# Tomsk-Smart-Tech/video-stream-segmenetation

Measured on AMD Instinct MI355X. Metric: frames/sec (640×480, batch=8) at 1/2/4/8 MI355X + mask max-abs-err vs ref, higher is better.
Workload: dtype bf16; 1 GPU; 8 synthetic 640x480 RGB u8 frames per GPU per step (resident in HBM) -> 256x144 f32 masks, 4 steps in flight (one handle, 4 slots, 4 streams); global_batch=8, frame=640x480x3, model_res=256x144, pw_gemm=v_mfma_f32_16x16x32_bf16, f32 activations split hi+lo, graph=True, inflight=4, parallelism=dp1

## Files before the change

### video-stream-segmenetation_amd/csrc/vss_kernels.h

```cpp
#pragma once
#include <cstddef>
#include <cstdint>

#include <hip/hip_runtime.h>

namespace vss {

enum Prec : int { PREC_F32 = 0, PREC_BF16X2 = 1, PREC_BF16 = 2 };

enum BlockMode : int { MODE_IR_EXPAND = 0, MODE_IR_DIRECT = 1, MODE_DEC = 2 };

__host__ __device__ constexpr int block_flags(int norm_in, int residual, int xp, int sp, int ks, int stem_in = 0) {
  return (norm_in ? 1 : 0) | (residual ? 2 : 0) | ((xp - 1) << 2) | ((sp - 1) << 4) | ((ks - 1) << 6) |
         (stem_in ? 256 : 0);
}
__host__ __device__ constexpr bool flags_stem_in(int f) { return (f & 256) != 0; }
__host__ __device__ constexpr int flags_xp(int f) { return ((f >> 2) & 3) + 1; }
__host__ __device__ constexpr int flags_sp(int f) { return ((f >> 4) & 3) + 1; }
__host__ __device__ constexpr int flags_ks(int f) { return ((f >> 6) & 3) + 1; }

constexpr int kThreads = 256;
constexpr int kLdsGranule = 2048, kLdsGranulesPerCu = 80;
__host__ __device__ constexpr int lds_wg_per_cu(int bytes) {
  return kLdsGranulesPerCu / ((bytes + kLdsGranule - 1) / kLdsGranule);
}
constexpr int kMaxAcc = 16;
#ifndef VSS_PERM
#define VSS_PERM 0
#endif
#ifndef VSS_XS_PAD
#define VSS_XS_PAD 4
#endif
#ifndef VSS_HS1
#define VSS_HS1 20
#endif
#ifndef VSS_QUADS
#define VSS_QUADS 1
#endif
__host__ __device__ constexpr int block_pix(int r) { return VSS_PERM ? (r < 4 ? r : (r < 12 ? r + 4 : r - 8)) : r; }
__host__ __device__ constexpr int hid_stride(int stride) { return stride == 2 ? 20 : VSS_HS1; }

#ifndef VSS_SWZ
#define VSS_SWZ 1
#endif
__host__ __device__ constexpr int pow2div16(int q) {
  return q % 16 == 0 ? 16 : (q % 8 == 0 ? 8 : (q % 4 == 0 ? 4 : (q % 2 == 0 ? 2 : 1)));
}
__host__ __device__ constexpr int gray_swz(int pix, int m) { return (pix ^ (pix >> 1)) & (m - 1); }
constexpr int kAccSlots = 4;

__host__ __device__ constexpr int r4(int v) { return (v + 3) & ~3; }
__host__ __device__ constexpr int cmax(int a, int b) { return a > b ? a : b; }

__host__ __device__ constexpr int dw_run(int TW, int NPB, int PW) {
  return (TW % 4 == 0 && 16 % (TW / 4) == 0 && NPB % 4 == 0 && (NPB / 4) % PW == 0)   ? 4
         : (TW % 2 == 0 && 16 % (TW / 2) == 0 && NPB % 2 == 0 && (NPB / 2) % PW == 0) ? 2
                                                                                      : 1;
}

struct BlockLds {
  int IH, IW, P_in, P_in_pad, P_out, CX, XS, LD2, SR, SC;
  bool XQM;
  int XPL, XSW, HPL, RS, RSW, XRW;
  int NCB, NPB, NCHUNK, PW, CS, NPBW, NACC;
  int xt, xr, w1, w2, wdw, bdw, b2, wimg_end, lr, nrm, uc, work, stt, total;
  int slab_stride;
  int slab;
};

__host__ __device__ constexpr int stem_xwp(int IW) {
  if (!VSS_SWZ) return 2 * IW + 2;
  const int xw = 2 * IW + 1, hw2 = IW + 1;
  int x = xw;
  while ((x - hw2) % 32 != 0) ++x;
  return x;
}
__host__ __device__ constexpr int stem_in_lds(int IH, int IW) {
  return r4(3 * (2 * IH + 1) * stem_xwp(IW)) + 27 * 16 + 16;
}

__host__ __device__ constexpr BlockLds block_lds(int mode, int stride, int TH, int TW, int cin, int cskip, int chid,
                                                 int cout, int stem_in = 0) {
  BlockLds L{};
  L.IH = stride == 2 ? 2 * TH + 1 : TH + 2;
  L.IW = stride == 2 ? 2 * TW + 1 : TW + 2;
  L.P_in = L.IH * L.IW;
  L.P_in_pad = (L.P_in + 15) & ~15;
  L.P_out = TH * TW;
  L.CX = mode == 2  ? cin + cskip : cin;
  L.XQM = VSS_SWZ && mode == 1;
  L.XS = !VSS_SWZ ? L.CX + VSS_XS_PAD : (L.XQM ? 4 : (mode == 2 ? L.CX + (TW == 16 ? 8 : VSS_XS_PAD) : L.CX));
  L.XPL = L.XQM ? 4 * L.P_in_pad : 0;
  L.XSW = VSS_SWZ && mode == 0 ? pow2div16(L.CX / 4) : 1;

  L.RS = VSS_SWZ ? cout : cout + 4;
  L.RSW = VSS_SWZ ? pow2div16(cout / 4) : 1;
  L.XRW = VSS_SWZ ? pow2div16(cin / 4) : 1;
  L.LD2 = chid + 8;
  L.SR = (TH + 1) / 2 + 3;
  L.SC = (TW + 1) / 2 + 3;
  L.NCB = cout / 16;
  L.NPB = L.P_out / 16;
  L.NCHUNK = chid / 16;
  L.CS = L.NCHUNK >= 4 ? 4 : (L.NCHUNK >= 2 ? 2 : 1);
  L.PW = 4 / L.CS;
  L.NPBW = L.NPB / L.PW;
  L.NACC = L.NPBW * L.NCB;
  L.HPL = VSS_SWZ && mode == 0 && dw_run(TW, L.NPB, 1) == 1 ? 4 * (L.P_in_pad + (stride == 2 ? 1 : 0)) : 0;
  L.slab_stride = L.P_out * L.RS;
  const int xt_floats = L.XQM ? L.P_in_pad * L.CX : r4(L.P_in_pad * L.XS);
  int o = 0;
  L.xt = o;  o += xt_floats;
  L.xr = o;  o += (mode == 0 && stride == 1 && cin == cout) ? r4(L.P_out * cin) : 0;
  L.w1 = o;
  L.w2 = o;  o += mode == 0 ? 0 : r4(cout * L.LD2 / 2);
  L.wdw = o; o += mode == 0 ? 0 : r4(9 * chid);
  L.bdw = o; o += mode == 0 ? 0 : r4(chid);
  L.b2 = o;  o += r4(cout);
  L.wimg_end = o;
  const bool slab_in_xt = mode == 2 && L.CS * L.slab_stride <= xt_floats;
  const bool dec_quads = mode == 2 && VSS_QUADS && TH % 2 == 0 && TW % 2 == 0;
  L.work = o;
  L.lr = o;
  const int hid_floats = L.HPL ? 4 * 4 * L.HPL : 4 * L.P_in_pad * hid_stride(stride);
  o += cmax(cmax(cmax(mode == 0 ? hid_floats : 1024, slab_in_xt ? 0 : L.CS * L.slab_stride),
                 mode == 2 && !dec_quads ? r4(L.SR * L.SC * cin) : 0),
            stem_in ? stem_in_lds(L.IH, L.IW) : 0);
  L.nrm = o; o += mode == 2 ? r4(2 * cin) : 0;
  L.uc = o;  o += (mode == 2 && !dec_quads) ? 4 * L.P_in_pad : 0;
  L.slab = slab_in_xt ? L.xt : L.work;
  L.stt = slab_in_xt ? L.work : L.xt;
  L.total = o;
  return L;
}

struct ExpandFrag {
  int NK, NCB, aw, f4s, a2, bytes;
};
constexpr int kFragF4 = 11;
__host__ __device__ constexpr ExpandFrag expand_frag(int cin, int cout) {
  ExpandFrag F{};
  F.NK = cin / 16;
  F.NCB = cout / 16;
  F.aw = 0;
  F.f4s = F.aw + 512 * F.NK;
  F.a2 = F.f4s + kFragF4 * 64;
  F.bytes = F.a2 + 512 * F.NCB;
  return F;
}
__host__ __device__ constexpr int frag_off(int n, int i, int l) {
  return (n % 2 == 1 && i == n - 1) ? (n / 2) * 1024 + l * 8 : (i / 2) * 1024 + l * 16 + (i % 2) * 8;
}

#ifdef VSS_TRACE
#define VSS_TRACE_FIELD unsigned long long* trace;
#define VSS_STAMP(k)                                                                                  \
  do {                                                                                                \
    if constexpr (!COH) {                                                                             \
      if (threadIdx.x == 0 && p.trace) {                                                              \
        unsigned long long* t_ = p.trace + (((long)blockIdx.z * gridDim.y + blockIdx.y) * gridDim.x + blockIdx.x) * 16; \
        t_[(k)] = __builtin_amdgcn_s_memrealtime();                                                   \
        t_[8 + (k)] = __builtin_amdgcn_s_memtime();                                                   \
        if ((k) == 0) {                                                                               \
                                    \
          t_[7] = __builtin_amdgcn_s_getreg((31 << 11) | 4);                                          \
          t_[15] = __builtin_amdgcn_s_getreg((15 << 11) | 20);                                        \
        }                                                                                             \
      }                                                                                               \
    }                                                                                                 \
  } while (0)
#else
#define VSS_TRACE_FIELD
#define VSS_STAMP(k) \
  do {               \
  } while (0)
#endif

struct StemParams {
  const uint8_t* frames;
  long row_stride, frame_stride;
  int fh, fw, fc;
  int Hm, Wm;
  float ry, rx;
  const float* w;
  const float* b;
  float* y;
  int Ho, Wo, cout;
  unsigned long long* acc_zero;
  int acc_stride;
  VSS_TRACE_FIELD
};

struct BlockParams {
  const float* wimg;
  long wimg_stride;
  const char* wfrag;
// ... 440 lines not shown
```

### video-stream-segmenetation_amd/csrc/vss_kernels.hip

```cpp
#include <hip/hip_runtime.h>

#include <vector>

#include "vss_kernels.h"

namespace vss {

typedef float f4 __attribute__((ext_vector_type(4)));
typedef unsigned u4 __attribute__((ext_vector_type(4)));
typedef __bf16 bf4 __attribute__((ext_vector_type(4)));
typedef __bf16 bf8 __attribute__((ext_vector_type(8)));

__device__ __forceinline__ const void* uniform_ptr(const void* p) {
  const unsigned long long v = reinterpret_cast<unsigned long long>(p);
  const unsigned lo = __builtin_amdgcn_readfirstlane((unsigned)v);
  const unsigned hi = __builtin_amdgcn_readfirstlane((unsigned)(v >> 32));
  return reinterpret_cast<const void*>(((unsigned long long)hi << 32) | lo);
}

template <bool COH>
struct Gm {
  const float* b;
  __amdgpu_buffer_rsrc_t r;
  __device__ __forceinline__ explicit Gm(const float* base) : b(base) {
// ... 433 lines not shown
    }
  }
};

#ifndef VSS_WDMA
#define VSS_WDMA 1
#endif
#ifndef VSS_WDMA_ALL
#define VSS_WDMA_ALL 0
#endif
#ifndef VSS_WDMA_FIRST
#define VSS_WDMA_FIRST 0
#endif
constexpr bool block_wdma(int mode, int wimg_f4) {
  return VSS_WDMA && (VSS_WDMA_ALL || mode == 2 || wimg_f4 >= 2560);
}
template <int N>
__device__ __forceinline__ void dma_f4(const f4* src, f4* dst) {
  const int lane = (int)threadIdx.x & 63;
  const int wb = __builtin_amdgcn_readfirstlane(((int)threadIdx.x >> 6) * 64);
  for (int o = wb; o < N; o += 256)
    if (N % 64 == 0 || o + lane < N)
      __builtin_amdgcn_global_load_lds((__attribute__((address_space(1))) void*)(src + o + lane),
                                       (__attribute__((address_space(3))) void*)(dst + o), 16, 0, 0);
}
struct NoStaged {
  template <class Load>
  __device__ __forceinline__ void issue(Load) {}
  template <class Store>
  __device__ __forceinline__ void commit(Store) const {}
};
template <bool ON>
__device__ __forceinline__ void dma_wait() {
  if constexpr (ON) asm volatile("s_waitcnt vmcnt(0)" ::: "memory");
}

template <bool B>
struct ChunkTag {
  static constexpr bool value = B;
};

template <int MODE, int STRIDE, int TH, int TW, int CIN, int CSKIP, int CH, int COUT, int FLAGS, int PREC, bool COH>
__device__ __forceinline__ void block_body(const BlockParams& p, int bx, int by, int bz, float* smem) {
  constexpr bool STEM_IN = flags_stem_in(FLAGS);
  constexpr BlockLds L = block_lds(MODE, STRIDE, TH, TW, CIN, CSKIP, CH, COUT, STEM_IN);
  constexpr bool NORM_IN = (FLAGS & 1) != 0, RES = (FLAGS & 2) != 0;
  constexpr int XP = flags_xp(FLAGS), SP = flags_sp(FLAGS), KS = flags_ks(FLAGS);
  static_assert(KS == 1 || MODE == MODE_IR_EXPAND, "only expand layers split their hidden channels");
  static_assert(SP == 1 || MODE == MODE_DEC, "skip parts: decoder only");
  constexpr int IW = L.IW, P_IN = L.P_in, P_IN_PAD = L.P_in_pad, P_OUT = L.P_out, XS = L.XS;
  constexpr int NCB = L.NCB, NPB = L.NPB, NCHUNK = L.NCHUNK, PW = L.PW, CS = L.CS, NPBW = L.NPBW;
  constexpr int RS = L.RS, SS = L.slab_stride;
  static_assert(L.NACC <= kMaxAcc, "too many accumulators per wave");
  static_assert(CIN % 16 == 0 && CH % 16 == 0 && COUT % 16 == 0 && P_OUT % 16 == 0, "shape");
  static_assert(MODE != MODE_IR_EXPAND || CIN <= 64, "expand cin <= 64");
  static_assert(!RES || (STRIDE == 1 && CIN == COUT && MODE != MODE_DEC), "residual shape");
  static_assert(MODE != MODE_IR_EXPAND || CS == 4, "expand deals its chunks to the 4 waves");
  static_assert(NPB % PW == 0, "pixel blocks must split evenly over the wave groups");
  constexpr int XT_FLOATS = L.XQM ? P_IN_PAD * L.CX : r4(P_IN_PAD * XS);
  static_assert(MODE != MODE_DEC || (XT_FLOATS >= (NORM_IN ? kAccSlots * 2 * CIN * 2 : 0) &&
                                     (L.slab == L.xt ? L.stt == L.work : (L.stt == L.xt && XT_FLOATS >= 1024))),
                "decoder: xt holds the src's norm slots (prologue); the stats scratch (epilogue) sits in the "
                "work region when the slabs take xt, else in xt");
  const int tid = threadIdx.x, lane = tid & 63, wave = tid >> 6;
  const int r = lane & 15, g = lane >> 4;
  const int n = KS == 1 ? bz : bz / KS;
  const int ks = KS == 1 ? 0 : bz % KS;
  const int oy0 = by * TH, ox0 = bx * TW;
  const int iy0 = STRIDE * oy0 - 1, ix0 = STRIDE * ox0 - 1;
  const int Ho = p.Ho, Wo = p.Wo;
  float* xt = smem + L.xt;
  const uint16_t* w2s = reinterpret_cast<const uint16_t*>(smem + L.w2);
  const float* wdws = smem + L.wdw;
  const float* bdws = smem + L.bdw;
  const float* b2s = smem + L.b2;
  float* work = smem + L.work;
  float* slabs = smem + L.slab;
  float* stt = smem + L.stt;
  auto xq = [&](int pix, int q) {
    if constexpr (L.XQM) return q * L.XPL + 4 * pix;
    else return pix * XS + 4 * (q ^ gray_swz(pix, L.XSW));
  };
  auto sq = [&](int sl, int pix, int q) { return sl * SS + pix * RS + 4 * (q ^ gray_swz(pix, L.RSW)); };
  auto rq = [&](int pix, int q) { return pix * CIN + 4 * (q ^ (pix & (L.XRW - 1))); };
  constexpr bool EXPAND = MODE == MODE_IR_EXPAND;
  constexpr ExpandFrag F = expand_frag(CIN, COUT);
  const char* frag = EXPAND ? p.wfrag + ks * p.wfrag_stride : nullptr;
  const int wave_u = __builtin_amdgcn_readfirstlane(wave);
  FragRegs<EXPAND ? F.NK : 1> w1f;
  f4 b1f;
  auto load_w1 = [&](int ck) {
    const char* rec = frag + ck * F.bytes;
    w1f.load(rec + F.aw, lane);
    b1f = *reinterpret_cast<const f4*>(rec + F.f4s + g * 16);
  };
  VSS_STAMP(0);

  constexpr int WIMG_F4 = (L.wimg_end - L.w1) / 4;
  constexpr bool WDMA = block_wdma(MODE, WIMG_F4);
  const f4* wsrc = reinterpret_cast<const f4*>(p.wimg + ks * p.wimg_stride);
  f4* wdst = reinterpret_cast<f4*>(smem + L.w1);
  if constexpr (MODE == MODE_DEC) {
    constexpr int CL = CIN, C4L = CL / 4, SR = L.SR, SC = L.SC;
    const int h = p.H, w = p.W;
    float* lr = smem + L.lr;
    float* nrm = smem + L.nrm;
    const int sy0 = max(0, (oy0 - 1) / 2 - 1), sx0 = max(0, (ox0 - 1) / 2 - 1);
    const float* xn = p.x + (long)n * h * w * CL;
    const float* sn = p.skip + (long)n * Ho * Wo * CSKIP;
    constexpr int NSLOT16 = NORM_IN ? kAccSlots * 2 * CL / 2 : 0;
    Staged<NSLOT16> st_slots;
    const Gm<COH> g_slots(reinterpret_cast<const float*>(p.in_acc + (long)n * p.acc_stride));
    if constexpr (NORM_IN) st_slots.issue([&](int i) { return g_slots.ld(4L * i); });
    static_assert(CL % 16 == 0 && CSKIP % 16 == 0, "16-channel staging items");
    constexpr int GL = CL / 16, GS = CSKIP / 16;
    constexpr bool QUADS = VSS_QUADS && TH % 2 == 0 && TW % 2 == 0;
    constexpr int QH = L.IH / 2, QW = IW / 2, NQI = QH * QW * C4L, NQ = QUADS ? (NQI + 255) / 256 : 0;
    Staged16<QUADS ? 0 : SR * SC * GL, XP, VSS_STAGE16_DEC> st_lr;
    f4 tap[XP][NQ > 0 ? NQ : 1][4];
    Staged16<P_IN_PAD * GS, SP, VSS_STAGE16_DEC> st_sk;
    constexpr bool SKP = VSS_SWZ && GS == 1 && !L.XQM && VSS_STAGE16_DEC == 0 && (XS / 4) % 4 == 2;
    auto skip_pix = [&](int it) { return SKP ? (it & ~3) | ((it & 1) << 1) | ((it >> 1) & 1) : it; };
    std::conditional_t<WDMA, NoStaged, Staged<WIMG_F4>> st_w;
    {
      const float* xb[XP];
#pragma unroll
      for (int q = 0; q < XP; ++q) xb[q] = xn + q * p.x_part_stride;
      if constexpr (QUADS) {
        const int j0 = (iy0 - 1) / 2, i0 = (ix0 - 1) / 2;
#pragma unroll
        for (int k = 0; k < NQ; ++k) {
          const int it = min(tid + 256 * k, NQI - 1);
          const int c4 = it % C4L, qq = it / C4L, qx = qq % QW, qy = qq / QW;
          const int ya = min(max(j0 + qy, 0), h - 1), yb = min(max(j0 + qy + 1, 0), h - 1);
          const int ca = min(max(i0 + qx, 0), w - 1), cb = min(max(i0 + qx + 1, 0), w - 1);
          const unsigned o[4] = {(unsigned)((ya * w + ca) * CL + 4 * c4), (unsigned)((ya * w + cb) * CL + 4 * c4),
                                 (unsigned)((yb * w + ca) * CL + 4 * c4), (unsigned)((yb * w + cb) * CL + 4 * c4)};
#pragma unroll
          for (int q = 0; q < XP; ++q)
#pragma unroll
            for (int t = 0; t < 4; ++t)
              tap[q][k][t] = *reinterpret_cast<const f4*>(reinterpret_cast<const char*>(xb[q]) + (o[t] << 2));
        }
      } else {
        st_lr.issue(xb, [&](int i) {
          const int pr = i / GL, gq = i - pr * GL;
          const int yy = min(h - 1, sy0 + pr / SC), xx = min(w - 1, sx0 + pr % SC);
          return (unsigned)((yy * w + xx) * CL + 16 * gq);
        });
      }
      const float* sb[SP];
#pragma unroll
      for (int q = 0; q < SP; ++q) sb[q] = sn + q * p.skip_part_stride;
      st_sk.issue(sb, [&](int i) {
        const int pix = skip_pix(i / GS), gq = i - (i / GS) * GS, py = pix / IW;
        const int yy = min(max(iy0 + py, 0), Ho - 1), xx = min(max(ix0 + pix - py * IW, 0), Wo - 1);
        return (unsigned)((yy * Wo + xx) * CSKIP + 16 * gq);
      });
    }
    if constexpr (WDMA) dma_f4<WIMG_F4>(wsrc, reinterpret_cast<f4*>(smem + L.w1));
    st_w.issue([&](int i) { return wsrc[i]; });
    VSS_STAMP(6);
    static_assert(SR * SC * CL < 65536, "tap offsets are u16");
    unsigned* uc = reinterpret_cast<unsigned*>(smem + L.uc);
    if constexpr (!QUADS)
    for (int pix = tid; pix < P_IN_PAD; pix += 256) {
      const int yy = iy0 + pix / IW, xx = ix0 + pix % IW;
// ... 176 lines not shown
        const unsigned x1 = (unsigned)min(sp.fw - 1, (int)ceilf(fx));
        dxs[u][e] = fx - x0f;
        const unsigned o0 = (unsigned)x0f * (unsigned)sp.fc, o1 = x1 * (unsigned)sp.fc;
#pragma unroll
        for (int c = 0; c < 3; ++c) {
          raw[u][e][c] = __builtin_amdgcn_raw_buffer_load_b8(frsrc, (int)(t0 + o0) + c, 0, 0);
          raw[u][e][3 + c] = __builtin_amdgcn_raw_buffer_load_b8(frsrc, (int)(t0 + o1) + c, 0, 0);
          raw[u][e][6 + c] = __builtin_amdgcn_raw_buffer_load_b8(frsrc, (int)(t1 + o0) + c, 0, 0);
          raw[u][e][9 + c] = __builtin_amdgcn_raw_buffer_load_b8(frsrc, (int)(t1 + o1) + c, 0, 0);
        }
      }
    }
    VSS_STAMP(6);
#pragma unroll
    for (int u = 0; u < NR; ++u) {
      float o[2][3];
      prep_finish2(raw[u][0], raw[u][1], dys[u], dxs[u][0], dys[u], dxs[u][1], o[0], o[1]);
      const int ly = lys[u], yy = r0 + ly;
#pragma unroll
      for (int e = 0; e < 2; ++e) {
        const int lx = lxs[u] + e * HW2, xx = c0 + lx;
        const bool in = tid + 256 * u < NPAIR && lx < XW;
        const bool valid = ((unsigned)yy < (unsigned)sp.Hm) & ((unsigned)xx < (unsigned)sp.Wm);
        if (in) {
#pragma unroll
          for (int c = 0; c < 3; ++c) x0s[(c * XH + ly) * XWP + lx] = valid ? o[e][c] : 0.f;
        }
      }
    }
#pragma unroll
    for (int u = 0; u < 2; ++u) {
      const int i = tid + 256 * u;
      if (i < 27 * 16) sws[i] = wr[u];
    }
    if (tid < 16) sbs[tid] = sb;
    if (bx == 0 && by == 0)
      for (int i = tid; i < sp.acc_stride; i += 256) {
        if constexpr (COH)
          __hip_atomic_store(sp.acc_zero + (long)n * sp.acc_stride + i, 0ull, __ATOMIC_RELAXED, __HIP_MEMORY_SCOPE_AGENT);
        else
          sp.acc_zero[(long)n * sp.acc_stride + i] = 0ull;
      }
    st_w.commit([&](int i, f4 v) { wdst[i] = v; });
    VSS_STAMP(4);
    dma_wait<WDMA>();
    __syncthreads();
    VSS_STAMP(5);
    {
      const StemTaps taps = stem_taps<XH * XWP, XWP>(sws, r, g);
      if constexpr (VSS_SWZ) {
        const f4 bias4 = *reinterpret_cast<const f4*>(sbs + 4 * g);
        for (int blk = wave; blk < P_IN_PAD / 16; blk += 4) {
          const int pa = min(blk * 16 + r, P_IN - 1), py = pa / IW, px = pa - py * IW;
          const f4 acc = stem_mfma_t(taps, x0s + 2 * py * XWP + 2 * px, bias4);
          *reinterpret_cast<f4*>(xt + xq(blk * 16 + r, g)) = relu6v(acc);
        }
      } else {
        const float bias = sbs[r];
        for (int blk = wave; blk < P_IN_PAD / 16; blk += 4) {
          const int pa = min(blk * 16 + r, P_IN - 1), py = pa / IW, px = pa - py * IW;
          const f4 acc = stem_mfma(taps, x0s + 2 * py * XWP + 2 * px, bias);
          const int p0 = blk * 16 + 4 * g;
#pragma unroll
          for (int i = 0; i < 4; ++i) xt[xq(p0 + i, r >> 2) + (r & 3)] = relu6f(acc[i]);
        }
      }
      const bool interior = iy0 >= 0 && iy0 + L.IH <= H && ix0 >= 0 && ix0 + IW <= W;
      if (!interior) {
        __syncthreads();
        for (int i = tid; i < P_IN * 4; i += 256) {
          const int q = L.XQM ? i / P_IN : i & 3, e = L.XQM ? i - q * P_IN : i >> 2, qy = e / IW, qx = e - qy * IW;
          const int yy = iy0 + qy, xx = ix0 + qx;
          if (yy < 0 || yy >= H || xx < 0 || xx >= W)
            *reinterpret_cast<f4*>(xt + xq(qy * IW + qx, q)) = f4{0.f, 0.f, 0.f, 0.f};
        }
      }
    }

  } else {
    const int H = p.H, W = p.W;
    const float* xn = p.x + (long)n * H * W * CIN;
    static_assert(CIN % 16 == 0, "16-channel staging items");
    constexpr int GI = CIN / 16;
    Staged16<P_IN_PAD * GI, XP, VSS_STAGE16> st_x;
    std::conditional_t<WDMA, NoStaged, Staged<WIMG_F4>> st_w;
    if constexpr (WDMA && VSS_WDMA_FIRST) dma_f4<WIMG_F4>(wsrc, reinterpret_cast<f4*>(smem + L.w1));
    {
      const float* xb[XP];
#pragma unroll
      for (int q = 0; q < XP; ++q) xb[q] = xn + q * p.x_part_stride;
      st_x.issue(xb, [&](int i) {
        const int pix = i / GI, gq = i - pix * GI, py = pix / IW;
        const int yy = min(max(iy0 + py, 0), H - 1), xx = min(max(ix0 + pix - py * IW, 0), W - 1);
        return (unsigned)((yy * W + xx) * CIN + 16 * gq);
      });
    }
    if constexpr (WDMA && !VSS_WDMA_FIRST) dma_f4<WIMG_F4>(wsrc, reinterpret_cast<f4*>(smem + L.w1));
    st_w.issue([&](int i) { return wsrc[i]; });
    if constexpr (EXPAND) load_w1(wave_u);
    VSS_STAMP(6);
    st_x.commit_sum([&](int i, int k, f4 v) {
      const int pix = i / GI, c4 = (i - pix * GI) * 4 + k;
      if constexpr (MODE == MODE_IR_EXPAND) {
        *reinterpret_cast<f4*>(xt + xq(pix, c4)) = to_operand<PREC>(v);
        if constexpr (RES) {
          const int py = pix / IW, px = pix - py * IW;
          if (py >= 1 && py <= TH && px >= 1 && px <= TW)
            *reinterpret_cast<f4*>(smem + L.xr + rq((py - 1) * TW + px - 1, c4)) = v;
        }
      } else {
        const int py = pix / IW, px = pix % IW;
        const int yy = iy0 + py, xx = ix0 + px;
        const bool valid = pix < P_IN && yy >= 0 && yy < H && xx >= 0 && xx < W;
        *reinterpret_cast<f4*>(xt + xq(pix, c4)) = valid ? v : f4{0.f, 0.f, 0.f, 0.f};
      }
    });
    st_w.commit([&](int i, f4 v) { wdst[i] = v; });
    VSS_STAMP(4);
  }
  dma_wait<WDMA>();
  __syncthreads();
  VSS_STAMP(1);

  f4 acc[L.NACC];
  const int pw = wave % PW, cw = wave / PW;
  constexpr int XR = dw_run(TW, NPB, MODE == MODE_IR_EXPAND ? 1 : PW);
  static_assert(NPB % XR == 0 && NPBW % XR == 0, "dw runs");
  auto run_pix = [&](int sb, int j) {
    if constexpr (XR == 1) return sb * 16 + block_pix(r);
    else return (sb * (16 * XR / TW) + r / (TW / XR)) * TW + (r % (TW / XR)) * XR + j;
  };

  if constexpr (MODE == MODE_IR_EXPAND) {
    constexpr int HSD = hid_stride(STRIDE);
    float* hid = work + wave * (L.HPL ? 4 * L.HPL : P_IN_PAD * HSD);
    auto hq = [&](int pix, int q) {
      if constexpr (L.HPL != 0) return q * L.HPL + 4 * pix;
      else return pix * HSD + 4 * q;
    };
    constexpr int NK = CIN / 16;
    constexpr int NCBI = P_IN_PAD / 16;
    static_assert(NCBI <= 32, "one validity bit per input pixel block");
    unsigned vmask = ~0u;
    if (!(iy0 >= 0 && iy0 + L.IH <= p.H && ix0 >= 0 && ix0 + IW <= p.W)) {
      vmask = 0u;
#pragma unroll
      for (int cb = 0; cb < NCBI; ++cb) {
        const int pix = cb * 16 + r, py = pix / IW, yy = iy0 + py, xx = ix0 + pix - py * IW;
        vmask |= (yy >= 0 && yy < p.H && xx >= 0 && xx < p.W) ? 1u << cb : 0u;
      }
    }
    auto expand_chunk = [&](int ck, auto first) {
      constexpr bool FIRST = decltype(first)::value;
      const char* rec = frag + ck * F.bytes;
      f4 wk[9];
#pragma unroll
      for (int t = 0; t < 9; ++t) wk[t] = *reinterpret_cast<const f4*>(rec + F.f4s + (4 * (1 + t) + g) * 16);
      const f4 bb = *reinterpret_cast<const f4*>(rec + F.f4s + (4 * 10 + g) * 16);
      FragRegs<NCB> w2f;
      w2f.load(rec + F.a2, lane);
      typename AFrag<PREC>::T aw[NK];
#pragma unroll
      for (int s = 0; s < NK; ++s) aw[s] = frag_a<PREC>(w1f.v[s]);
      const f4 bias = b1f;
      constexpr int UNRL = block_lds(MODE, STRIDE, TH, TW, CIN, CSKIP, CH, COUT, STEM_IN).P_in_pad / 16 <= 6
                               ? block_lds(MODE, STRIDE, TH, TW, CIN, CSKIP, CH, COUT, STEM_IN).P_in_pad / 16
                               : 2;
#pragma unroll UNRL
      for (int cb = 0; cb < NCBI; ++cb) {
        const int pix = cb * 16 + r;
        f4 d = bias;
#pragma unroll
        for (int s = 0; s < NK; ++s) d = mma16_op<PREC>(d, aw[s], *reinterpret_cast<const f4*>(xt + xq(pix, 4 * s + g)));
        *reinterpret_cast<f4*>(hid + hq(pix, g)) = clampv(d, (vmask >> cb) & 1u ? 6.f : 0.f);
      }
      wave_sync();
      {
        if constexpr (NCHUNK > 4) load_w1(min(ck + 4, NCHUNK - 1));
        typename AFrag<PREC>::T a2[NCB];
#pragma unroll
        for (int cb = 0; cb < NCB; ++cb) a2[cb] = frag_a<PREC>(w2f.v[cb]);
#pragma unroll
        for (int q = 0; q < NPB / XR; ++q) {
          const int pix0 = run_pix(q, 0), ly = pix0 / TW, lx0 = pix0 % TW;
          f4 a[XR];
#pragma unroll
          for (int j = 0; j < XR; ++j) a[j] = bb;
#pragma unroll
          for (int ky = 0; ky < 3; ++ky) {
            constexpr int NT = STRIDE * (XR - 1) + 3;
            f4 t[NT];
#pragma unroll
            for (int u = 0; u < NT; ++u)
              t[u] = *reinterpret_cast<const f4*>(hid + hq((STRIDE * ly + ky) * IW + STRIDE * lx0 + u, g));
#pragma unroll
            for (int j = 0; j < XR; ++j)
#pragma unroll
              for (int kx = 0; kx < 3; ++kx) a[j] = __builtin_elementwise_fma(wk[ky * 3 + kx], t[STRIDE * j + kx], a[j]);
          }
#pragma unroll
          for (int j = 0; j < XR; ++j) {
            const f4 b = to_operand<PREC>(relu6v(a[j]));
#pragma unroll
            for (int cb = 0; cb < NCB; ++cb) {
              f4& ac = acc[(q * XR + j) * NCB + cb];
              if constexpr (FIRST)
                ac = mma16_op<PREC>(f4{0.f, 0.f, 0.f, 0.f}, a2[cb], b);
              else
                ac = mma16_op<PREC>(ac, a2[cb], b);
            }
          }
        }
      }
      wave_sync();
    };
    static_assert(NCHUNK >= 4, "every wave has a first chunk");
    expand_chunk(wave_u, ChunkTag<true>{});
    for (int ck = wave_u + 4; ck < NCHUNK; ck += 4) expand_chunk(ck, ChunkTag<false>{});
  } else {
    auto dw_chunk = [&](int ck, auto first) {
      constexpr bool FIRST = decltype(first)::value;
      const int c0 = ck << 4;
      f4 wk[9];
#pragma unroll
      for (int t = 0; t < 9; ++t) wk[t] = *reinterpret_cast<const f4*>(wdws + t * CH + c0 + 4 * g);
      const f4 bb = *reinterpret_cast<const f4*>(bdws + c0 + 4 * g);
      typename AFrag<PREC>::T a2[NCB];
#pragma unroll
      for (int cb = 0; cb < NCB; ++cb) a2[cb] = lds_a<PREC>(w2s, L.LD2, cb * 16 + r, c0 + 4 * g);
#pragma unroll
      for (int q = 0; q < NPBW / XR; ++q) {
        const int pix0 = run_pix(pw + q * PW, 0), ly = pix0 / TW, lx0 = pix0 % TW;
        f4 a[XR];
#pragma unroll
        for (int j = 0; j < XR; ++j) a[j] = bb;
#pragma unroll
        for (int ky = 0; ky < 3; ++ky) {
          f4 t[XR + 2];
#pragma unroll
          for (int u = 0; u < XR + 2; ++u)
            t[u] = *reinterpret_cast<const f4*>(xt + xq((ly + ky) * IW + lx0 + u, (c0 >> 2) + g));
#pragma unroll
          for (int j = 0; j < XR; ++j)
#pragma unroll
            for (int kx = 0; kx < 3; ++kx) a[j] = __builtin_elementwise_fma(wk[ky * 3 + kx], t[j + kx], a[j]);
        }
#pragma unroll
        for (int j = 0; j < XR; ++j) {
          if constexpr (MODE == MODE_IR_DIRECT) a[j] = relu6v(a[j]);
          const f4 b = to_operand<PREC>(a[j]);
#pragma unroll
          for (int cb = 0; cb < NCB; ++cb) {
            f4& ac = acc[(q * XR + j) * NCB + cb];
            if constexpr (FIRST)
              ac = mma16_op<PREC>(f4{0.f, 0.f, 0.f, 0.f}, a2[cb], b);
            else
              ac = mma16_op<PREC>(ac, a2[cb], b);
          }
        }
      }
    };
    static_assert(CS <= NCHUNK, "every wave has a first chunk");
    dw_chunk(cw, ChunkTag<true>{});
    for (int ck = cw + CS; ck < NCHUNK; ck += CS) dw_chunk(ck, ChunkTag<false>{});
  }

  if constexpr (MODE == MODE_IR_DIRECT && CS == 1) {
    VSS_STAMP(2);
    const Gm<COH> gy(p.y + (long)n * Ho * Wo * COUT);
#pragma unroll
    for (int q = 0; q < NPBW / XR; ++q)
#pragma unroll
      for (int j = 0; j < XR; ++j) {
        const int pix = run_pix(pw + q * PW, j), ly = pix / TW, lx = pix % TW;
        const int oy = oy0 + ly, ox = ox0 + lx;
#pragma unroll
        for (int cb = 0; cb < NCB; ++cb) {
          f4 v = acc[(q * XR + j) * NCB + cb] + *reinterpret_cast<const f4*>(b2s + cb * 16 + 4 * g);
          if constexpr (RES) v = v + *reinterpret_cast<const f4*>(xt + xq((ly + 1) * IW + lx + 1, cb * 4 + g));
          if (oy < Ho && ox < Wo) gy.st(((long)oy * Wo + ox) * COUT + cb * 16 + 4 * g, v);
        }
      }
  } else {
  __syncthreads();
  VSS_STAMP(2);
  {
#pragma unroll
    for (int q = 0; q < NPBW / XR; ++q)
#pragma unroll
      for (int j = 0; j < XR; ++j)
#pragma unroll
        for (int cb = 0; cb < NCB; ++cb)
          *reinterpret_cast<f4*>(slabs + sq(cw, run_pix(pw + q * PW, j), cb * 4 + g)) = acc[(q * XR + j) * NCB + cb];
  }
  __syncthreads();
  constexpr int C4O = COUT / 4, NOUT = (P_OUT * C4O + 255) / 256;
  const Gm<COH> gy(p.y + ks * p.y_part_stride + (long)n * Ho * Wo * COUT);
  f4 outv[MODE == MODE_DEC ? NOUT : 1];
#pragma unroll
  for (int k = 0; k < NOUT; ++k) {
    const int i = tid + 256 * k;
    if (i < P_OUT * C4O) {
      const int pix = i / C4O, c4 = i % C4O;
      const int ly = pix / TW, lx = pix % TW;
      const int oy = oy0 + ly, ox = ox0 + lx;
      const bool valid = oy < Ho && ox < Wo;
      f4 v = *reinterpret_cast<const f4*>(slabs + sq(0, pix, c4));
#pragma unroll
      for (int s = 1; s < CS; ++s) v = v + *reinterpret_cast<const f4*>(slabs + sq(s, pix, c4));
      if (KS == 1 || ks == 0) {
        v = v + *reinterpret_cast<const f4*>(b2s + 4 * c4);
        if constexpr (RES) {
          if constexpr (MODE == MODE_IR_EXPAND)
            v = v + *reinterpret_cast<const f4*>(smem + L.xr + rq(pix, c4));
          else
            v = v + *reinterpret_cast<const f4*>(xt + xq((ly + 1) * IW + lx + 1, c4));
        }
      }
      if constexpr (MODE == MODE_DEC) {
        outv[k] = v;
        *reinterpret_cast<f4*>(slabs + sq(0, pix, c4)) = valid ? v : f4{0.f, 0.f, 0.f, 0.f};
      } else if (valid) {
        gy.st(((long)oy * Wo + ox) * COUT + 4 * c4, v);
      }
    }
  }
  if constexpr (MODE == MODE_DEC) {
    __syncthreads();
    constexpr int G = 256 / COUT;
    static_assert((P_OUT + G - 1) / G <= 16, "f64 lane sums: at most 16 terms (bound above)");
    long long* st64 = reinterpret_cast<long long*>(stt);
    const int c = tid % COUT, gg = tid / COUT;
    if (gg < G) {
      double s = 0.0, q = 0.0;
#pragma unroll
      for (int pix = 0; pix < P_OUT; pix += G) {
        if (pix + gg < P_OUT) {
          const float v = slabs[sq(0, pix + gg, c >> 2) + (c & 3)];
          s += (double)__builtin_rintf(v * 0x1p32f);
          q += (double)__builtin_rintf(v * v * 0x1p24f);
        }
      }
      constexpr double kBias = 0x1.8p52;
      long long si = __double_as_longlong(s + kBias) - __double_as_longlong(kBias);
      long long qi = __double_as_longlong(q + kBias) - __double_as_longlong(kBias);
      if (q >= 0x1p51) {
        asm volatile("" ::: "memory");
        si = 0;
        qi = 0;
        for (int pix = 0; pix < P_OUT; pix += G) {
          if (pix + gg < P_OUT) {
            const float v = slabs[sq(0, pix + gg, c >> 2) + (c & 3)];
            si += (long long)__builtin_rintf(v * 0x1p32f);
            qi += (long long)__builtin_rintf(v * v * 0x1p24f);
          }
        }
      }
      st64[gg * COUT + c] = si;
      st64[256 + gg * COUT + c] = qi;
    }
    __syncthreads();
    if (tid < 2 * COUT) {
      const int base = tid < COUT ? tid : 256 + (tid - COUT);
      long long t = 0;
#pragma unroll
      for (int k = 0; k < G; ++k) t += st64[base + k * COUT];
      const int slot = (by * p.tiles_x + bx) % kAccSlots;
      __hip_atomic_fetch_add(p.out_acc + (long)n * p.acc_stride + slot * 2 * COUT + tid, (unsigned long long)t,
                             __ATOMIC_RELAXED, __HIP_MEMORY_SCOPE_AGENT);
    }
#pragma unroll
    for (int k = 0; k < NOUT; ++k) {
      const int i = tid + 256 * k;
      if (i < P_OUT * C4O) {
        const int pix = i / C4O, c4 = i % C4O;
        const int oy = oy0 + pix / TW, ox = ox0 + pix % TW;
        if (oy < Ho && ox < Wo) gy.st(((long)oy * Wo + ox) * COUT + 4 * c4, outv[k]);
      }
    }
  }
  }
  if constexpr (STEM_IN) {
    const Gm<COH> gst(p.stem.y + (long)n * p.H * p.W * 16);
    for (int i = tid; p.stem.y != nullptr && i < TH * TW * 4; i += 256) {
      const int pix = i >> 2, q = i & 3;
      const int yy = oy0 + pix / TW, xx = ox0 + pix % TW;
      if (yy < p.H && xx < p.W)
        gst.st(((long)yy * p.W + xx) * 16 + 4 * q,
               *reinterpret_cast<const f4*>(xt + xq((pix / TW + 1) * IW + pix % TW + 1, q)));
    }
  }
  VSS_STAMP(3);
}

constexpr int block_min_waves(int mode, int stride, int th, int tw, int cin, int cout, int prec) {
  if (mode != MODE_IR_EXPAND) return 1;
  const BlockLds L = block_lds(mode, stride, th, tw, cin, 0, 64, cout);
  if (tw != 8 || L.P_out > 32 || L.P_in_pad > 96 || L.NPB * L.NCB > 6) return 1;
  return prec == PREC_F32 ? (cin == 16 ? 4 : 3) : (cin == 16 ? 5 : 4);
}

template <int MODE, int STRIDE, int TH, int TW, int CIN, int CSKIP, int CH, int COUT, int FLAGS, int PREC>
__global__ __launch_bounds__(256) __attribute__((amdgpu_waves_per_eu(block_min_waves(MODE, STRIDE, TH, TW, CIN, COUT, PREC))))
void k_block(BlockParams p) {
  extern __shared__ __attribute__((aligned(16))) float smem[];
  const TileIdx t = xcd_tile();
  block_body<MODE, STRIDE, TH, TW, CIN, CSKIP, CH, COUT, FLAGS, PREC, false>(p, t.x, t.y, t.z, smem);
}

template <int TH, int TW, int PREC>
__global__ __launch_bounds__(kWideThreads) void k_stem_b1(BlockParams p) {
  extern __shared__ __attribute__((aligned(16))) float smem[];
  constexpr int WT = kWideThreads, NWAVE = WT / 64;
  constexpr StemB1Lds S = stem_b1_lds(TH, TW);
  constexpr int IH = S.IH, IW = S.IW, P_IN = S.P_IN, P_IN_PAD = S.P_IN_PAD, XS = S.XS;
  constexpr int XH = S.XH, XW = S.XW, XWP = S.XWP, NX = (XH * XW + WT - 1) / WT;
  constexpr BlockLds B = block_lds(MODE_IR_DIRECT, 1, TH, TW, 16, 0, 16, 16, 1);
  constexpr int WIMG4 = (B.wimg_end - B.w1) / 4;
  static_assert(WIMG4 <= WT && 27 * 16 <= WT, "one weight element per thread");
  float* x0s = smem + S.x0;
  float* sws = smem + S.sw;
  float* sbs = smem + S.sb;
  float* xt = smem + S.xt;
  float* wim = smem + S.wim;
  const TileIdx tl = xcd_tile();
  const int bx = tl.x, by = tl.y, n = tl.z;
  const int tid = threadIdx.x, lane = tid & 63, wave = tid >> 6, r = lane & 15, g = lane >> 4;
  const int oy0 = by * TH, ox0 = bx * TW, iy0 = oy0 - 1, ix0 = ox0 - 1;
  const StemParams& sp = p.stem;
  const int H = p.H, W = p.W;
  const uint8_t* fr = sp.frames + (long)n * sp.frame_stride;
  const int r0 = 2 * iy0 - 1, c0 = 2 * ix0 - 1;
  const f4 wv = reinterpret_cast<const f4*>(p.wimg)[min(tid, WIMG4 - 1)];
  const float swr = sp.w[min(tid, 27 * 16 - 1)];
  const float sb = sp.b[min(tid, 15)];
  uint32_t raw[NX][12];
  float dys[NX], dxs[NX];
#pragma unroll
  for (int u = 0; u < NX; ++u) {
    const int i = min(tid + WT * u, XH * XW - 1);
    const int ly = i / XW, lx = i - ly * XW;
    const int yy = min(max(r0 + ly, 0), sp.Hm - 1), xx = min(max(c0 + lx, 0), sp.Wm - 1);
    const PrepTap t = prep_tap(fr, sp.row_stride, sp.fc, sp.fh, sp.fw, sp.ry, sp.rx, yy, xx);
    prep_load(t, raw[u]);
    dys[u] = t.dy;
    dxs[u] = t.dx;
  }
  float o[NX][3];
#pragma unroll
  for (int u = 0; u < NX; u += 2) {
    if (u + 1 < NX)
      prep_finish2(raw[u], raw[u + 1], dys[u], dxs[u], dys[u + 1], dxs[u + 1], o[u], o[u + 1]);
    else
      prep_finish(raw[u], dys[u], dxs[u], o[u]);
  }
#pragma unroll
  for (int u = 0; u < NX; ++u) {
    const int i = tid + WT * u;
    if (i < XH * XW) {
      const int ly = i / XW, lx = i - ly * XW;
      const int yy = r0 + ly, xx = c0 + lx;
      const bool valid = yy >= 0 && yy < sp.Hm && xx >= 0 && xx < sp.Wm;
#pragma unroll
      for (int c = 0; c < 3; ++c) x0s[(c * XH + ly) * XWP + lx] = valid ? o[u][c] : 0.f;
    }
  }
  if (tid < WIMG4) reinterpret_cast<f4*>(wim)[tid] = wv;
  if (tid < 27 * 16) sws[(tid % 27) * 16 + tid / 27] = swr;
  if (tid < 16) sbs[tid] = sb;
  if (bx == 0 && by == 0)
    for (int i = tid; i < sp.acc_stride; i += WT) sp.acc_zero[(long)n * sp.acc_stride + i] = 0ull;
  __syncthreads();
  {
    const StemTaps taps = stem_taps<XH * XWP, XWP>(sws, r, g);
    const float bias = sbs[r];
    const bool interior = iy0 >= 0 && iy0 + IH <= H && ix0 >= 0 && ix0 + IW <= W;
    for (int blk = wave; blk < P_IN_PAD / 16; blk += NWAVE) {
      const int pa = min(blk * 16 + r, P_IN - 1), py = pa / IW, px = pa - py * IW;
      const f4 acc = stem_mfma(taps, x0s + 2 * py * XWP + 2 * px, bias);
      const int p0 = blk * 16 + 4 * g;
// ... 201 lines not shown
```

Baseline: 246,800 frames/s.

## Load expand-block residual from global into registers instead of LDS copy

Removes the LDS residual copy (xr region) in expand blocks and instead loads the residual input directly from global memory into registers before the final sync, summing partial XP parts. The input tile in LDS is sized to the unpadded pixel count for expand mode, with the tail pixels of the last partial MMA block remapped to earlier valid pixels. These cuts LDS footprint, which may allow more workgroups per CU. A specific stride-2 6x8 f32 config also gets a waves-per-EU hint of 4. The cost is extra global reads and register pressure for the held residual values.

```diff
diff --git a/video-stream-segmenetation_amd/csrc/vss_kernels.h b/video-stream-segmenetation_amd/csrc/vss_kernels.h
--- a/video-stream-segmenetation_amd/csrc/vss_kernels.h
+++ b/video-stream-segmenetation_amd/csrc/vss_kernels.h
@@ -61,9 +61,9 @@
 struct BlockLds {
   int IH, IW, P_in, P_in_pad, P_out, CX, XS, LD2, SR, SC;
   bool XQM;
-  int XPL, XSW, HPL, RS, RSW, XRW;
+  int XPL, XSW, HPL, RS, RSW;
   int NCB, NPB, NCHUNK, PW, CS, NPBW, NACC;
-  int xt, xr, w1, w2, wdw, bdw, b2, wimg_end, lr, nrm, uc, work, stt, total;
+  int xt, w1, w2, wdw, bdw, b2, wimg_end, lr, nrm, uc, work, stt, total;
   int slab_stride;
   int slab;
 };
@@ -95,7 +95,6 @@
 
   L.RS = VSS_SWZ ? cout : cout + 4;
   L.RSW = VSS_SWZ ? pow2div16(cout / 4) : 1;
-  L.XRW = VSS_SWZ ? pow2div16(cin / 4) : 1;
   L.LD2 = chid + 8;
   L.SR = (TH + 1) / 2 + 3;
   L.SC = (TW + 1) / 2 + 3;
@@ -108,10 +107,9 @@
   L.NACC = L.NPBW * L.NCB;
   L.HPL = VSS_SWZ && mode == 0 && dw_run(TW, L.NPB, 1) == 1 ? 4 * (L.P_in_pad + (stride == 2 ? 1 : 0)) : 0;
   L.slab_stride = L.P_out * L.RS;
-  const int xt_floats = L.XQM ? L.P_in_pad * L.CX : r4(L.P_in_pad * L.XS);
+  const int xt_floats = L.XQM ? L.P_in_pad * L.CX : r4((mode == 0 ? L.P_in : L.P_in_pad) * L.XS);
   int o = 0;
   L.xt = o;  o += xt_floats;
-  L.xr = o;  o += (mode == 0 && stride == 1 && cin == cout) ? r4(L.P_out * cin) : 0;
   L.w1 = o;
   L.w2 = o;  o += mode == 0 ? 0 : r4(cout * L.LD2 / 2);
   L.wdw = o; o += mode == 0 ? 0 : r4(9 * chid);
diff --git a/video-stream-segmenetation_amd/csrc/vss_kernels.hip b/video-stream-segmenetation_amd/csrc/vss_kernels.hip
--- a/video-stream-segmenetation_amd/csrc/vss_kernels.hip
+++ b/video-stream-segmenetation_amd/csrc/vss_kernels.hip
@@ -539,7 +539,6 @@
     else return pix * XS + 4 * (q ^ gray_swz(pix, L.XSW));
   };
   auto sq = [&](int sl, int pix, int q) { return sl * SS + pix * RS + 4 * (q ^ gray_swz(pix, L.RSW)); };
-  auto rq = [&](int pix, int q) { return pix * CIN + 4 * (q ^ (pix & (L.XRW - 1))); };
   constexpr bool EXPAND = MODE == MODE_IR_EXPAND;
   constexpr ExpandFrag F = expand_frag(CIN, COUT);
   const char* frag = EXPAND ? p.wfrag + ks * p.wfrag_stride : nullptr;
@@ -882,7 +881,7 @@
     const float* xn = p.x + (long)n * H * W * CIN;
     static_assert(CIN % 16 == 0, "16-channel staging items");
     constexpr int GI = CIN / 16;
-    Staged16<P_IN_PAD * GI, XP, VSS_STAGE16> st_x;
+    Staged16<(EXPAND ? P_IN : P_IN_PAD) * GI, XP, VSS_STAGE16> st_x;
     std::conditional_t<WDMA, NoStaged, Staged<WIMG_F4>> st_w;
     if constexpr (WDMA && VSS_WDMA_FIRST) dma_f4<WIMG_F4>(wsrc, reinterpret_cast<f4*>(smem + L.w1));
     {
@@ -903,11 +902,6 @@
       const int pix = i / GI, c4 = (i - pix * GI) * 4 + k;
       if constexpr (MODE == MODE_IR_EXPAND) {
         *reinterpret_cast<f4*>(xt + xq(pix, c4)) = to_operand<PREC>(v);
-        if constexpr (RES) {
-          const int py = pix / IW, px = pix - py * IW;
-          if (py >= 1 && py <= TH && px >= 1 && px <= TW)
-            *reinterpret_cast<f4*>(smem + L.xr + rq((py - 1) * TW + px - 1, c4)) = v;
-        }
       } else {
         const int py = pix / IW, px = pix % IW;
         const int yy = iy0 + py, xx = ix0 + px;
@@ -969,9 +963,11 @@
 #pragma unroll UNRL
       for (int cb = 0; cb < NCBI; ++cb) {
         const int pix = cb * 16 + r;
+        static_assert(P_IN % 16 == 0 || P_IN > 32, "a partial last block has two blocks before it");
+        const int xpix = P_IN % 16 != 0 && pix >= P_IN ? pix - 32 : pix;
         f4 d = bias;
 #pragma unroll
-        for (int s = 0; s < NK; ++s) d = mma16_op<PREC>(d, aw[s], *reinterpret_cast<const f4*>(xt + xq(pix, 4 * s + g)));
+        for (int s = 0; s < NK; ++s) d = mma16_op<PREC>(d, aw[s], *reinterpret_cast<const f4*>(xt + xq(xpix, 4 * s + g)));
         *reinterpret_cast<f4*>(hid + hq(pix, g)) = clampv(d, (vmask >> cb) & 1u ? 6.f : 0.f);
       }
       wave_sync();
@@ -1082,6 +1078,24 @@
         }
       }
   } else {
+  constexpr int C4O = COUT / 4, NOUT = (P_OUT * C4O + 255) / 256;
+  constexpr bool RES_X = RES && MODE == MODE_IR_EXPAND;
+  f4 resv[RES_X ? NOUT : 1][XP];
+  if constexpr (RES_X) {
+    if (KS == 1 || ks == 0) {
+      const float* xn = p.x + (long)n * p.H * p.W * CIN;
+#pragma unroll
+      for (int k = 0; k < NOUT; ++k) {
+        const int i = min(tid + 256 * k, P_OUT * C4O - 1);
+        const int pix = i / C4O, c4 = i % C4O, ly = pix / TW;
+        const int oy = min(oy0 + ly, p.H - 1), ox = min(ox0 + pix - ly * TW, p.W - 1);
+        const unsigned o = (unsigned)((oy * p.W + ox) * CIN + 4 * c4) << 2;
+#pragma unroll
+        for (int q = 0; q < XP; ++q)
+          resv[k][q] = *reinterpret_cast<const f4*>(reinterpret_cast<const char*>(xn + q * p.x_part_stride) + o);
+      }
+    }
+  }
   __syncthreads();
   VSS_STAMP(2);
   {
@@ -1094,7 +1108,6 @@
           *reinterpret_cast<f4*>(slabs + sq(cw, run_pix(pw + q * PW, j), cb * 4 + g)) = acc[(q * XR + j) * NCB + cb];
   }
   __syncthreads();
-  constexpr int C4O = COUT / 4, NOUT = (P_OUT * C4O + 255) / 256;
   const Gm<COH> gy(p.y + ks * p.y_part_stride + (long)n * Ho * Wo * COUT);
   f4 outv[MODE == MODE_DEC ? NOUT : 1];
 #pragma unroll
@@ -1111,9 +1124,12 @@
       if (KS == 1 || ks == 0) {
         v = v + *reinterpret_cast<const f4*>(b2s + 4 * c4);
         if constexpr (RES) {
-          if constexpr (MODE == MODE_IR_EXPAND)
-            v = v + *reinterpret_cast<const f4*>(smem + L.xr + rq(pix, c4));
-          else
+          if constexpr (MODE == MODE_IR_EXPAND) {
+            f4 x = resv[k][0];
+#pragma unroll
+            for (int q = 1; q < XP; ++q) x = x + resv[k][q];
+            v = v + x;
+          } else
             v = v + *reinterpret_cast<const f4*>(xt + xq((ly + 1) * IW + lx + 1, c4));
         }
       }
@@ -1196,6 +1212,7 @@
 constexpr int block_min_waves(int mode, int stride, int th, int tw, int cin, int cout, int prec) {
   if (mode != MODE_IR_EXPAND) return 1;
   const BlockLds L = block_lds(mode, stride, th, tw, cin, 0, 64, cout);
+  if (stride == 2 && th == 6 && tw == 8 && cin == 16 && prec == PREC_F32) return 4;
   if (tw != 8 || L.P_out > 32 || L.P_in_pad > 96 || L.NPB * L.NCB > 6) return 1;
   return prec == PREC_F32 ? (cin == 16 ? 4 : 3) : (cin == 16 ? 5 : 4);
 }
```

Measured after the change: 247,400 frames/s, median of 4. No clear change (+0.3%).
